# luicalrob/Triangulation-in-Deformable-Scenes

Measured on AMD Instinct MI355X. Metric: LM iterations/sec + ms/iter at 100k corr × 2 views; 1/2/4/8-GPU scaling, higher is better.
Workload: dtype f64

## Files before the change

### triangulation-in-deformable-scenes_amd/csrc/spcg.hip

```cpp
#include <hip/hip_runtime.h>

#include <algorithm>
#include <cstdio>
#include <type_traits>

#include "spcg.h"
#include "ticket.h"
#include "wave.h"

namespace deftri {
namespace sp {

using wv::wave_sum;
using wv::wave_max;

__device__ __forceinline__ double block_sum(double v, double *red4) {
    const int lane = threadIdx.x & 63, w = threadIdx.x >> 6;
    v = wave_sum(v);
    if (lane == 0) red4[w] = v;
    __syncthreads();
    const double s = (red4[0] + red4[1]) + (red4[2] + red4[3]);
    __syncthreads();
    return s;
}

__device__ __forceinline__ double pval(const double2 *__restrict__ zp, double beta, int64_t i) {
    const double2 v = zp[i];
    return __fma_rn(beta, v.y, v.x);
}

__device__ __forceinline__ int it_state(const SpDev &G, int it, double &beta) {
    beta = 0.0;
    if (G.rec[0] != 0.0) return (int)G.rec[0];
    const double *rk = G.red + (int64_t)kSpRed * it;
    if (rk[2] != 0.0) return (int)rk[2];
    if (rk[1] <= G.tol2 * G.red[1]) return kSpConverged;
    if (it >= G.max_it) return kSpBudget;
    if (it > 0) beta = rk[0] / G.red[(int64_t)kSpRed * (it - 1)];
    return 0;
}

__device__ __forceinline__ void record_stop(const SpDev &G, int it, int st) {
    if (G.rec[0] == 0.0) {
        G.rec[0] = st;
        G.rec[1] = it;
    }
}

__host__ __device__ __forceinline__ int row_grid(int nrb) { return 8 * ((max(nrb, 1) + 7) / 8); }
__device__ __forceinline__ int row_block(int b, int nrb) {
    const int seg = (max(nrb, 1) + 7) / 8;
    return (b & 7) * seg + (b >> 3);
}

__device__ __forceinline__ int heavy_dof(const SpDev &G, int h) { return h < G.Q ? 6 * h : 6 * G.Q + (h - G.Q); }

__device__ __forceinline__ bool gated_off(const int *g) { return g && !*g; }
__device__ __forceinline__ double lam_of(const SpDev &G, double lam) { return G.lam_dev ? *G.lam_dev : lam; }

__device__ __forceinline__ void publish(double *p, double v) { st_sc1(p, v); }
__device__ __forceinline__ double fetch(const double *p) {
    return ld_sc1(p);
}

__device__ __forceinline__ int tri3(int a, int b) { return a * (a + 1) / 2 + b; }
__device__ __forceinline__ int tri6(int a, int b) { return a * (a + 1) / 2 + b; }

template <class JT, int GU>
__global__ void __launch_bounds__(256) __attribute__((amdgpu_waves_per_eu(GU == 4 ? 5 : GU == 6 ? 4 : 1, GU == 4 ? 5 : GU == 6 ? 4 : 3)))
k_sp_glin_rows(const SpDev G, JT *__restrict__ pj) {
    __shared__ double red4[4];
    if (gated_off(G.lgate)) return;
    const int lb = row_block(blockIdx.x, G.nrb2);
    const int w = lb * 4 + (threadIdx.x >> 6), lane = threadIdx.x & 63;
    double mx = 0.0;
    if (w < G.nwaves) {
        const int l = G.rowmap[64 * w + lane];
        double D[6] = {0, 0, 0, 0, 0, 0}, bb[3] = {0, 0, 0};
        if (l >= 0) {
            for (int j = G.rep_off[l]; j < G.rep_off[l + 1]; j++) {
                const double *J = G.Jr + 6 * (int64_t)j;
                const double wt = G.Wr[j];
#pragma unroll
                for (int r = 0; r < 2; r++) {
                    const double er = G.Er[2 * (int64_t)j + r];
#pragma unroll
                    for (int a = 0; a < 3; a++) {
                        const double ja = J[3 * r + a] * wt;
#pragma unroll
                        for (int c = 0; c <= a; c++) D[tri3(a, c)] += ja * J[3 * r + c];
                        bb[a] -= J[3 * r + a] * (wt * er);
                    }
                }
            }
            const int d0 = G.dep_off[l], d1 = G.dep_off[l + 1];
            for (int jb = d0; jb < d1; jb += 4) {
                double Jb[4][4], wb[4], eb[4];
#pragma unroll
                for (int u = 0; u < 4; u++) {
                    const int64_t j = jb + u < d1 ? jb + u : jb;
#pragma unroll
                    for (int c = 0; c < 4; c++) Jb[u][c] = G.Jd[4 * j + c];
                    wb[u] = G.Wd[j];
                    eb[u] = G.Ed[j];
                }
#pragma unroll
                for (int u = 0; u < 4; u++) {
                    if (jb + u >= d1) break;
                    const int64_t j = jb + u;
                    const double *J = Jb[u];
                    const double wt = wb[u], er = eb[u];
#pragma unroll
                    for (int a = 0; a < 3; a++) {
                        const double ja = J[a] * wt;
#pragma unroll
                        for (int c = 0; c <= a; c++) D[tri3(a, c)] += ja * J[c];
                        bb[a] -= J[a] * (wt * er);
                        G.cdep[3 * j + a] = ja * J[3];
                    }
                    G.wss[j] = (J[3] * wt) * J[3];
                }
            }
        }
        double H[6];
#pragma unroll
        for (int k = 0; k < 6; k++) H[k] = D[k];
        const int64_t n = G.nslots * 64;
        struct Raw { double j0, j1, j2, w, x; };
        const double *__restrict__ Ja = G.Ja, *__restrict__ Wa = G.Wa, *__restrict__ Ea = G.Ea;
        const double *__restrict__ Jd = G.Jd, *__restrict__ Wd = G.Wd;
        const int64_t jld = G.jld;
        const bool w1 = G.Q == 1 && G.pinfo != nullptr;
        auto load = [&](int m) -> Raw {
            const bool dep = m <= -2;
            const int mm = max(m, 0), jj = max(-2 - m, 0);
            const double *pa = Ja + (int64_t)(3 * (mm & 3)) * jld + (mm >> 2);
            const double *pd = Jd + 4 * (int64_t)jj;
            const double *Jc = dep ? pd : pa;
            const int64_t st = dep ? 1 : jld;
            const double *W = dep ? Wd + jj : w1 ? G.pinfo : Wa + (mm >> 2);
            const double *X = dep ? pd + 3 : Ea + (mm >> 2);
            return Raw{Jc[0], Jc[st], Jc[2 * st], *W, *X};
        };
        auto value = [&](int m, const Raw &r, double *v, double &wt, double &er) {
            const bool arap = m >= 0, dep = m <= -2;
            v[0] = dep ? (r.j0 * r.w) * r.x : arap ? r.j0 : 0.0;
            v[1] = dep ? (r.j1 * r.w) * r.x : arap ? r.j1 : 0.0;
            v[2] = dep ? (r.j2 * r.w) * r.x : arap ? r.j2 : 0.0;
            wt = arap ? r.w : 0.0;
            er = arap ? r.x : 0.0;
        };
        auto add = [&](const double *v, double wt, double er) {
#pragma unroll
            for (int a = 0; a < 3; a++) {
                const double ja = v[a] * wt;
#pragma unroll
                for (int c = 0; c <= a; c++) H[tri3(a, c)] += ja * v[c];
                bb[a] -= v[a] * (wt * er);
            }
        };
        int64_t k = G.woff[w] * 64 + lane;
        const int64_t k1 = G.woff[w + 1] * 64 + lane;
        auto step = [&](auto U_, bool clamp) {
            constexpr int U = decltype(U_)::value;
            int m[U];
            int64_t kk[U];
            bool in[U];
            Raw r[U];
#pragma unroll
            for (int u = 0; u < U; u++) {
                in[u] = !clamp || k + 64 * u < k1;
                kk[u] = in[u] ? k + 64 * u : k1 - 64;
            }
#pragma unroll
            for (int u = 0; u < U; u++) m[u] = G.pmap[kk[u]];
#pragma unroll
            for (int u = 0; u < U; u++) r[u] = load(m[u]);
#pragma unroll
            for (int u = 0; u < U; u++) {
                double v[3], wt, er;
                value(m[u], r[u], v, wt, er);
                if (!in[u]) wt = er = 0.0;
                add(v, wt, er);
                if (pj)
#pragma unroll
                    for (int a = 0; a < 3; a++) pj[a * n + kk[u]] = (JT)v[a];
            }
            k += U * 64;
        };
        using I4 = std::integral_constant<int, 4>;
        if constexpr (GU == 4) {
            while (k + 3 * 64 < k1) step(I4{}, false);
        } else if constexpr (GU == 6) {
            while (k + 5 * 64 < k1) step(std::integral_constant<int, 6>{}, false);
            if (k + 4 * 64 < k1) step(std::integral_constant<int, 6>{}, true);
        } else {
            while (k + 7 * 64 < k1) step(std::integral_constant<int, 8>{}, false);
            if (k + 4 * 64 < k1) step(std::integral_constant<int, 8>{}, true);
        }
        if (k < k1) step(I4{}, true);
        if (G.wsplit[w]) {
#pragma unroll
            for (int k = 0; k < 6; k++) H[k] += __shfl_xor(H[k], 32);
#pragma unroll
            for (int a = 0; a < 3; a++) bb[a] += __shfl_xor(bb[a], 32);
        }
        if (l >= 0) {
#pragma unroll
            for (int k = 0; k < 6; k++) { G.Hv[6 * (int64_t)l + k] = H[k]; G.Dv[6 * (int64_t)l + k] = D[k]; }
            const int64_t o = G.hd + 3 * (int64_t)(G.row0 + l);
#pragma unroll
            for (int a = 0; a < 3; a++) G.b[o + a] = bb[a];
            mx = fmax(fabs(H[0]), fmax(fabs(H[2]), fabs(H[5])));
        }
    }
    mx = wave_max(mx);
    if ((threadIdx.x & 63) == 0) red4[threadIdx.x >> 6] = mx;
    __syncthreads();
    if (threadIdx.x == 0 && lb < max(G.nrb2, 1)) G.mpart[lb] = fmax(fmax(red4[0], red4[1]), fmax(red4[2], red4[3]));
}

__global__ void __launch_bounds__(256) k_sp_glin_blocks(const SpDev G) {
    __shared__ double red[kSpLin][4];
    if (gated_off(G.lgate)) return;
    const int2 gr = G.glb[blockIdx.x];
    const int4 d = G.blk[gr.x];
    const int kind = d.x & 0xff, owned = d.x >> 8;
    const int lane = threadIdx.x & 63, w = threadIdx.x >> 6;
    const int i = d.z + threadIdx.x;
    double *out = G.lpart + (int64_t)kSpLin * gr.x;
    if (kind == SP_ARAP) {
        if (!owned) return;
        double a[kSpLin];
#pragma unroll
        for (int k = 0; k < kSpLin; k++) a[k] = 0.0;
        const int iend = G.blk[gr.x + gr.y - 1].w;
        for (int ii = i; ii < iend; ii += 256) {
            double J[6];
#pragma unroll
            for (int r = 0; r < 6; r++) J[r] = G.Ja[(12 + r) * G.jld + ii];
            const double wv = G.Wa[ii], er = G.Ea[ii];
#pragma unroll
            for (int r = 0; r < 6; r++) {
                const double jr = J[r] * wv;
#pragma unroll
                for (int c = 0; c <= r; c++) a[tri6(r, c)] += jr * J[c];
                a[21 + r] -= J[r] * (wv * er);
            }
        }
        for (int k = threadIdx.x; k < kSpLin * (gr.y - 1); k += 256) out[kSpLin + k] = 0.0;
#pragma unroll
        for (int k = 0; k < kSpLin; k++) {
            const double v = wave_sum(a[k]);
            if (lane == 0) red[k][w] = v;
        }
        __syncthreads();
        if (threadIdx.x < kSpLin) {
            const int k = threadIdx.x;
            out[k] = (red[k][0] + red[k][1]) + (red[k][2] + red[k][3]);
        }
    } else {
        double h = 0.0, bs = 0.0;
        if (i < d.w) {
            const int le = G.dperm[i];
            const double js = G.Jd[4 * (int64_t)le + 3];
            h = G.wss[le];
            bs = -js * (G.Wd[le] * G.Ed[le]);
        }
        h = wave_sum(h);
        bs = wave_sum(bs);
        if (lane == 0) { red[0][w] = h; red[1][w] = bs; }
        __syncthreads();
        if (threadIdx.x < 2) {
            const int k = threadIdx.x;
            out[k] = (red[k][0] + red[k][1]) + (red[k][2] + red[k][3]);
        }
    }
}

__global__ void __launch_bounds__(256) k_sp_glin_heavy(const SpDev G) {
    __shared__ double lds[8][32];
    __shared__ int last;
    if (gated_off(G.lgate)) return;
    const int ch = blockIdx.x, h = G.ch_h[ch];
    const int dim = h < G.Q ? kSpLin : 2;
    const int c = threadIdx.x & 31, g = threadIdx.x >> 5;
    double acc = 0.0;
    if (c < dim) {
        int64_t k = G.ch_lo[ch] + g;
        const int64_t k1 = G.ch_lo[ch + 1];
        for (; k + 7 * 8 < k1; k += 64) {
            double v[8];
#pragma unroll
            for (int u = 0; u < 8; u++) v[u] = G.lpart[(int64_t)kSpLin * G.hv_blk[k + 8 * u] + c];
#pragma unroll
            for (int u = 0; u < 8; u++) acc += v[u];
        }
        for (; k < k1; k += 8) acc += G.lpart[(int64_t)kSpLin * G.hv_blk[k] + c];
    }
    lds[g][c] = acc;
    __syncthreads();
    if ((int)threadIdx.x < dim) {
        double t = 0.0;
#pragma unroll
        for (int gg = 0; gg < 8; gg++) t += lds[gg][threadIdx.x];
        publish(G.chpart + (int64_t)kSpLin * ch + threadIdx.x, t);
    }
    const int c0 = G.hch_off[h], c1 = G.hch_off[h + 1];
    if (threadIdx.x == 0) {
        __atomic_signal_fence(__ATOMIC_SEQ_CST);
        __builtin_amdgcn_s_waitcnt(0);
        __atomic_signal_fence(__ATOMIC_SEQ_CST);
        last = __hip_atomic_fetch_add(G.hcnt + h, 1, __ATOMIC_RELAXED, __HIP_MEMORY_SCOPE_AGENT) == c1 - c0 - 1;
    }
    __syncthreads();
    if (!last) return;
    acc = 0.0;
    if (c < dim)
        for (int j = c0 + g; j < c1; j += 8) acc += fetch(G.chpart + (int64_t)kSpLin * j + c);
    __syncthreads();
    lds[g][c] = acc;
    __syncthreads();
    if ((int)threadIdx.x < dim) {
        double t = 0.0;
#pragma unroll
        for (int gg = 0; gg < 8; gg++) t += lds[gg][threadIdx.x];
        const int q = threadIdx.x;
        if (h < G.Q) {
            if (q < 21) G.hl[21 * (int64_t)h + q] = t;
            else G.b[6 * (int64_t)h + q - 21] = t;
        } else {
            if (q == 0) G.hl[21 * (int64_t)G.Q + (h - G.Q)] = t;
            else G.b[6 * (int64_t)G.Q + (h - G.Q)] = t;
        }
    }
    if (threadIdx.x == 0) st_sc1(G.hcnt + h, 0);
}

__global__ void __launch_bounds__(256) k_sp_maxdiag(const SpDev G, double *out, int stage) {
    __shared__ double red4[4];
    if (gated_off(G.lgate)) return;
    double m = 0.0;
    if (stage == 0) {
        for (int i = threadIdx.x; i < G.nrb2; i += 256) m = fmax(m, G.mpart[i]);
    } else {
        for (int h = threadIdx.x; h < G.Q; h += 256)
#pragma unroll
            for (int a = 0; a < 6; a++) m = fmax(m, fabs(G.hl[21 * (int64_t)h + tri6(a, a)]));
        for (int s = threadIdx.x; s < G.S; s += 256) m = fmax(m, fabs(G.hl[21 * (int64_t)G.Q + s]));
    }
    m = wave_max(m);
    if ((threadIdx.x & 63) == 0) red4[threadIdx.x >> 6] = m;
    __syncthreads();
    if (threadIdx.x == 0) {
        const double v = fmax(fmax(red4[0], red4[1]), fmax(red4[2], red4[3]));
        out[0] = stage == 0 ? v : fmax(out[0], v);
    }
}

__global__ void k_sp_cvt_j(const double *__restrict__ J, float *__restrict__ J32, int64_t n, const int *gate) {
    if (gated_off(gate)) return;
    const int64_t i = (int64_t)blockIdx.x * 256 + threadIdx.x;
    if (i < n) J32[i] = (float)J[i];
}

__device__ __forceinline__ bool inv3(const double *A, double lam, double *M) {
    const double a00 = A[0] + lam, a10 = A[1], a11 = A[2] + lam, a20 = A[3], a21 = A[4], a22 = A[5] + lam;
    if (!(a00 > 0.0)) return false;
    const double l00 = sqrt(a00), l10 = a10 / l00, l20 = a20 / l00;
    const double d1 = a11 - l10 * l10;
    if (!(d1 > 0.0)) return false;
    const double l11 = sqrt(d1), l21 = (a21 - l20 * l10) / l11;
    const double d2 = a22 - l20 * l20 - l21 * l21;
    if (!(d2 > 0.0)) return false;
    const double l22 = sqrt(d2);
    const double i00 = 1.0 / l00, i11 = 1.0 / l11, i22 = 1.0 / l22;
    const double i10 = -l10 * i00 * i11;
    const double i21 = -l21 * i11 * i22;
    const double i20 = -(l20 * i00 + l21 * i10) * i22;
    M[0] = i00 * i00 + i10 * i10 + i20 * i20;
    M[1] = i11 * i10 + i21 * i20;
    M[2] = i11 * i11 + i21 * i21;
    M[3] = i22 * i20;
    M[4] = i22 * i21;
    M[5] = i22 * i22;
    return true;
}

__device__ __forceinline__ void mul3(const double *M, const double r[3], double z[3]) {
    z[0] = M[0] * r[0] + M[1] * r[1] + M[3] * r[2];
    z[1] = M[1] * r[0] + M[2] * r[1] + M[4] * r[2];
    z[2] = M[3] * r[0] + M[4] * r[1] + M[5] * r[2];
}

__device__ bool inv6(const double *Hl, double lam, double *Mo) {
    double L[36];
    for (int i = 0; i < 6; i++)
        for (int j = 0; j < 6; j++) L[i * 6 + j] = j <= i ? Hl[tri6(i, j)] + (i == j ? lam : 0.0) : 0.0;
    for (int j = 0; j < 6; j++) {
        double s = L[j * 6 + j];
        for (int k = 0; k < j; k++) s -= L[j * 6 + k] * L[j * 6 + k];
        if (!(s > 0.0)) return false;
        s = sqrt(s);
        L[j * 6 + j] = s;
        for (int i = j + 1; i < 6; i++) {
            double t = L[i * 6 + j];
            for (int k = 0; k < j; k++) t -= L[i * 6 + k] * L[j * 6 + k];
            L[i * 6 + j] = t / s;
        }
    }
    for (int c = 0; c < 6; c++) {
        double y[6];
        for (int i = 0; i < 6; i++) {
            double t = i == c ? 1.0 : 0.0;
            for (int k = 0; k < i; k++) t -= L[i * 6 + k] * y[k];
            y[i] = t / L[i * 6 + i];
        }
        for (int i = 5; i >= 0; i--) {
            double t = y[i];
            for (int k = i + 1; k < 6; k++) t -= L[k * 6 + i] * y[k];
// ... 845 lines not shown
                double z = 0.0;
                for (int c = 0; c < dim; c++) z += M[a * dim + c] * r[c];
                G.zp[o + a] = make_double2(z, p[a]);
                rz += r[a] * z;
                rr += r[a] * r[a];
            }
        }
        if (!G.include_heavy) rz = rr = 0.0;
    }
    rz = wave_sum(rz);
    rr = wave_sum(rr);
    if (lane == 0) { red[0][wv] = rz; red[1][wv] = rr; }
    __syncthreads();
    if (t == 0) {
        double s0 = 0.0, s1 = 0.0;
#pragma unroll
        for (int k = 0; k < nw; k++) { s0 += red[0][k]; s1 += red[1][k]; }
        double *out = G.upart + 2 * slot;
        if (G.fuse) {
            st_sc1(out, s0);
            st_sc1(out + 1, s1);
        } else {
            out[0] = s0;
            out[1] = s1;
        }
    }
    if (G.fuse && last_block(G, G.cnt + 16)) {
        __syncthreads();
        if (t < 256) dots_block(G, it + 1, dred);
    }
}

__global__ void __launch_bounds__(3 * kSpUpdRows) k_sp_update_sd(int it, const SpDev G, double lam, int tail) {
    __shared__ double sM[6 * kSpUpdRows], sR[3 * kSpUpdRows];
    __shared__ double red[2][3 * kSpUpdRows / 64];
    if (gated_off(G.gate) || G.rec[0] != 0.0) return;
    lam = lam_of(G, lam);
    const double gamma = G.xb[0], rr = G.xb[1], delta = G.xb[2];
    const double rr0 = it == 0 ? rr : G.red[1];
    double beta = 0.0, alpha = 0.0;
    int st = 0;
    if (rr <= G.tol2 * rr0) st = kSpConverged;
    else if (it >= G.max_it) st = kSpBudget;
    else {
        double den = delta;
        if (it > 0) {
            beta = gamma / G.red[(int64_t)kSpRed * (it - 1)];
            den = delta - beta * gamma / G.red[(int64_t)kSpRed * (it - 1) + 3];
        }
        alpha = gamma / den;
        if (!(den > 0.0) || !isfinite(alpha) || !isfinite(beta)) st = kSpBreakdown;
    }
    const int t = threadIdx.x, lane = t & 63, wv = t >> 6;
    if (blockIdx.x == 0 && t == 0) {
        double *rk = G.red + (int64_t)kSpRed * it;
        rk[0] = gamma; rk[1] = rr; rk[3] = alpha; rk[4] = delta;
        if (st) record_stop(G, it, st);
    }
    if (st || tail) return;
    constexpr int nw = 3 * kSpUpdRows / 64;
    double rz = 0.0, rr1 = 0.0;
    const int rb = (int)blockIdx.x - 1, slot = rb < 0 ? G.nrb : rb;
    if (rb >= 0) {
        const int l0 = rb * kSpUpdRows;
        const int nrow = min(kSpUpdRows, G.nown - l0);
        const int64_t o0 = G.hd + 3 * (int64_t)(G.row0 + l0);
        const bool on = t < 3 * nrow;
        double z = 0.0, pp = 0.0, w = 0.0, sp = 0.0, x = 0.0, r = 0.0;
        if (on) {
            const double2 v = G.zp[o0 + t];
            z = v.x; pp = v.y;
            w = G.q[o0 + t];
            if (G.tile) {
                const int l = l0 + t / 3, a = t - 3 * (t / 3);
                for (int k = G.txoff[l]; k < G.txoff[l + 1]; k++) w += G.xc[3 * (int64_t)k + a];
            }
            sp = G.sv[o0 + t];
            x = G.x[o0 + t];
            r = G.r[o0 + t];
        }
        const double *Mg = G.Mv + 6 * (int64_t)l0;
        if (t < 6 * nrow) sM[t] = Mg[t];
        if (t + 3 * kSpUpdRows < 6 * nrow) sM[t + 3 * kSpUpdRows] = Mg[t + 3 * kSpUpdRows];
        const double p = it > 0 ? z + beta * pp : z;
        const double s_ = it > 0 ? w + beta * sp : w;
        x += alpha * p;
        r -= alpha * s_;
        sR[t] = r;
        __syncthreads();
        if (on) {
            const int row = t / 3, a = t - 3 * row;
            const double *M = sM + 6 * row, *rv = sR + 3 * row;
            const int i0 = a == 0 ? 0 : a == 1 ? 1 : 3, i1 = a == 0 ? 1 : a == 1 ? 2 : 4, i2 = a == 0 ? 3 : a == 1 ? 4 : 5;
            const double zn = M[i0] * rv[0] + M[i1] * rv[1] + M[i2] * rv[2];
            G.x[o0 + t] = x;
            G.r[o0 + t] = r;
            G.sv[o0 + t] = s_;
            G.zp[o0 + t] = make_double2(zn, p);
            sd_send(G, l0 + row, a, zn, p);
            rz = r * zn;
            rr1 = r * r;
        }
    } else if (t < 256) {
        for (int h = t; h < G.Q + G.S; h += 256) {
            const int o = heavy_dof(G, h);
            const int dim = h < G.Q ? 6 : 1;
            double r[6], p[6];
            for (int a = 0; a < dim; a++) {
                const double2 v = G.zp[o + a];
                const double w = G.xb[3 + o + a] + lam * v.x;
                p[a] = it > 0 ? v.x + beta * v.y : v.x;
                const double s_ = it > 0 ? w + beta * G.sv[o + a] : w;
                G.sv[o + a] = s_;
                G.x[o + a] += alpha * p[a];
                r[a] = G.r[o + a] - alpha * s_;
                G.r[o + a] = r[a];
            }
            const double *M = h < G.Q ? G.Mh + 36 * (int64_t)h : G.Mh + 36 * (int64_t)G.Q + (h - G.Q);
            for (int a = 0; a < dim; a++) {
                double z = 0.0;
                for (int c = 0; c < dim; c++) z += M[a * dim + c] * r[c];
                G.zp[o + a] = make_double2(z, p[a]);
                rz += r[a] * z;
                rr1 += r[a] * r[a];
            }
        }
        if (!G.include_heavy) rz = rr1 = 0.0;
    }
    rz = wave_sum(rz);
    rr1 = wave_sum(rr1);
    if (lane == 0) { red[0][wv] = rz; red[1][wv] = rr1; }
    __syncthreads();
    if (t == 0) {
        double s0 = 0.0, s1 = 0.0;
#pragma unroll
        for (int k = 0; k < nw; k++) { s0 += red[0][k]; s1 += red[1][k]; }
        G.upart[2 * slot] = s0;
        G.upart[2 * slot + 1] = s1;
    }
}

__device__ __forceinline__ double shfl_up_d(double v, int d) {
    int2 p = __builtin_bit_cast(int2, v);
    p.x = __shfl_up(p.x, (unsigned)d, 64);
    p.y = __shfl_up(p.y, (unsigned)d, 64);
    return __builtin_bit_cast(double, p);
}

__device__ __forceinline__ int tile_state(const SpDev &G, int it, double &beta, double (*red)[4]) {
    beta = 0.0;
    __shared__ double s_r0;
    const double *rk = G.red + (int64_t)kSpRed * it;
    const double sw = rk[2], rr0 = G.red[1], gprev = it > 0 ? G.red[(int64_t)kSpRed * (it - 1)] : 1.0;
    if (threadIdx.x == 0) s_r0 = G.rec[0];
    __syncthreads();
    const double r0 = s_r0;
    if (r0 != 0.0) return (int)r0;
    const int n2 = it == 0 ? G.nrb + 1 : G.m_nh + row_grid(G.nrb);
    const double2 *parts = reinterpret_cast<const double2 *>(it == 0 ? G.upart : G.m2part);
    double a0 = 0.0, a1 = 0.0;
    int j = (int)threadIdx.x;
    for (; j + 3 * 256 < n2; j += 4 * 256) {
        double2 v[4];
#pragma unroll
        for (int u = 0; u < 4; u++) v[u] = parts[j + 256 * u];
#pragma unroll
        for (int u = 0; u < 4; u++) { a0 += v[u].x; a1 += v[u].y; }
    }
    for (; j < n2; j += 256) {
        const double2 v = parts[j];
        a0 += v.x;
        a1 += v.y;
    }
    const int lane = threadIdx.x & 63, w = threadIdx.x >> 6;
    a0 = wave_sum(a0);
    a1 = wave_sum(a1);
    if (lane == 0) { red[0][w] = a0; red[1][w] = a1; }
    __syncthreads();
    const double s0 = (red[0][0] + red[0][1]) + (red[0][2] + red[0][3]);
    const double s1 = (red[1][0] + red[1][1]) + (red[1][2] + red[1][3]);
    __syncthreads();
    int st = 0;
    if (sw != 0.0) st = (int)sw;
    else if (s1 <= G.tol2 * (it == 0 ? s1 : rr0)) st = kSpConverged;
    else if (it >= G.max_it) st = kSpBudget;
    if (blockIdx.x == 0 && threadIdx.x == 0) {
        G.red[(int64_t)kSpRed * it] = s0;
        G.red[(int64_t)kSpRed * it + 1] = s1;
        if (st) record_stop(G, it, st);
    }
    if (!st && it > 0) beta = s0 / gprev;
    return st;
}

__device__ __forceinline__ double tile_heavy_sum(const SpDev &G, int h, double *lds, bool coherent = false) {
    const int nb = G.t_grid - 1;
    const int dim = h < G.Q ? 6 : 1;
    const int c = threadIdx.x & 7, g = threadIdx.x >> 3;
    double acc = 0.0;
    if (G.tmulti) {
        const int q = h < G.Q ? h : (h - G.Q) >> 1, off = h < G.Q ? 0 : 6 + ((h - G.Q) & 1);
        const int seg = (G.ntile + 7) / 8, t1 = G.tpoff[q + 1];
        if (c < dim)
            for (int t = G.tpoff[q] + g; t < t1; t += 32) {
                const double *p = G.part + (int64_t)kSpPart * (8 * (t % seg) + t / seg) + off + c;
                acc += coherent ? fetch(p) : *p;
            }
    } else if (c < dim) {
        const int off = h < G.Q ? 0 : 6 + (h - G.Q);
        int k = g;
        for (; k + 7 * 32 < nb; k += 8 * 32) {
            double v[8];
#pragma unroll
            for (int u = 0; u < 8; u++) {
                const double *q = G.part + (int64_t)kSpPart * (k + 32 * u) + off + c;
                v[u] = coherent ? fetch(q) : *q;
            }
#pragma unroll
            for (int u = 0; u < 8; u++) acc += v[u];
        }
        for (; k < nb; k += 32) {
            const double *q = G.part + (int64_t)kSpPart * k + off + c;
            acc += coherent ? fetch(q) : *q;
        }
    }
    lds[threadIdx.x] = acc;
    __syncthreads();
    double t = 0.0;
    if ((int)threadIdx.x < dim)
        for (int gg = 0; gg < 32; gg++) t += lds[8 * gg + threadIdx.x];
    return t;
}

template <class JT, int SD = 0>
__global__ void __launch_bounds__(256) k_sp_tile(int it, const SpDev G, const JT *__restrict__ Jarap, double lam) {
    extern __shared__ double lds[];
    __shared__ double red[9][4];
    if (gated_off(G.gate)) return;
    lam = lam_of(G, lam);
    const int b = G.p1list ? G.p1list[blockIdx.x] : (int)blockIdx.x, tid = (int)threadIdx.x, lane = tid & 63, wv = tid >> 6;
    const bool heavy_wg = b == G.t_grid - 1;
    const int seg = (G.ntile + 7) / 8;
    const int t = heavy_wg ? G.ntile : (b & 7) * seg + (b >> 3);
    int r0 = 0, nr = 0, nh = 0, e0 = 0, ne = 0, h0 = 0, ns = 0, tq = 0;
    auto own_row = [&](int i) { return G.tmulti ? (G.trow[r0 + i] & 0x7fffffff) : G.row0 + r0 + i; };
    double2 zpre[3] = {make_double2(0.0, 0.0), make_double2(0.0, 0.0), make_double2(0.0, 0.0)};
    double2 zpre2[3] = {make_double2(0.0, 0.0), make_double2(0.0, 0.0), make_double2(0.0, 0.0)};
    double2 hz = make_double2(0.0, 0.0);
    uint2 mA = make_uint2(0u, 0u), mB = mA;
    int2 cA = make_int2(0, 0), cB = cA;
    int rsi = 0, dj0 = 0, dj1 = 0;
    int dsc0 = -1;
    double cd0[3] = {0.0, 0.0, 0.0}, ws0 = 0.0, Dp[6] = {0, 0, 0, 0, 0, 0};
    if (t < G.ntile) {
        const int32_t *T = G.ttab + 8 * (int64_t)t;
        r0 = T[0]; nr = T[1]; nh = T[2]; e0 = T[3]; ne = T[4]; h0 = T[5]; ns = T[6]; tq = T[7];
        if (tid < nr + nh) {
            const int row = tid < nr ? own_row(tid) : G.thalo[h0 + tid - nr];
            const int64_t o = G.hd + 3 * (int64_t)row;
#pragma unroll
            for (int c = 0; c < 3; c++) zpre[c] = G.zp[o + c];
        }
        if (tid + 256 < nr + nh) {
            const int i = tid + 256;
            const int row = i < nr ? own_row(i) : G.thalo[h0 + i - nr];
            const int64_t o = G.hd + 3 * (int64_t)row;
#pragma unroll
            for (int c = 0; c < 3; c++) zpre2[c] = G.zp[o + c];
        }
        const int hdof = tid < 6 ? 6 * tq + tid : 6 * G.Q + 2 * tq + tid - 6;
        if (tid < 8 && hdof < G.hd) hz = G.zp[hdof];
        const int64_t k0 = (int64_t)e0 + tid;
        if (tid < ne) { mA = G.tmeta[k0]; cA = G.tchunk[k0 >> 6]; }
        if (tid + 256 < ne) { mB = G.tmeta[k0 + 256]; cB = G.tchunk[(k0 + 256) >> 6]; }
        if (tid < nr) {
            const int l = G.tmulti ? own_row(tid) : r0 + tid;
            rsi = G.trs[r0 + tid];
            if (G.tmulti) {
                const int tdv = G.tdep[r0 + tid];
                if (tdv >= 0) {
                    const int jd = tdv >> 1;
                    dsc0 = tdv & 1;
#pragma unroll
                    for (int c = 0; c < 3; c++) cd0[c] = G.cdep[3 * (int64_t)jd + c];
                    ws0 = G.wss[jd];
                }
                if (G.trow[r0 + tid] < 0)
#pragma unroll
                    for (int kk = 0; kk < 6; kk++) Dp[kk] = G.Dv[6 * (int64_t)l + kk];
            } else {
                dj0 = G.dep_off[l];
                dj1 = G.dep_off[l + 1];
            }
        }
    }
    double beta;
    if (G.sd) {
        beta = 0.0;
        if (G.rec[0] != 0.0) return;
    } else if (G.tparts) {
        if (tile_state(G, it, beta, reinterpret_cast<double(*)[4]>(&red[0][0]))) return;
    } else if (it_state(G, it, beta)) {
        return;
    }
    double pap = 0.0, jts[6] = {0, 0, 0, 0, 0, 0}, sacc[2] = {0, 0};
    if (heavy_wg) {
        for (int64_t dd = tid; dd < G.hd; dd += 256) {
            const double p = pval(G.zp, beta, dd);
            G.ph[dd] = p;
            pap += lam * (p * p);
        }
        if (!G.include_heavy) pap = 0.0;
        pap = block_sum(pap, red[0]);
        if (tid == 0) G.m1part[b] = pap;
        return;
    }
    if (t < G.ntile) {
        double *pL = lds, *up = pL + 3 * (nr + nh), *rs = up + 3 * nr, *hp = rs + 3 * ns;
        const int64_t jld = G.jld;
        const uint64_t lt = (1ull << lane) - 1;
        if (tid < nr + nh)
#pragma unroll
            for (int c = 0; c < 3; c++) pL[3 * tid + c] = __fma_rn(beta, zpre[c].y, zpre[c].x);
        if (tid + 256 < nr + nh)
#pragma unroll
// ... 215 lines not shown
                    for (int u = 0; u < 4; u++)
                        if (j0 + u < ns)
#pragma unroll
                            for (int c = 0; c < 3; c++) q[c] += v[u][c];
                }
            }
            {
                const int k0 = G.txoff[l], k1 = G.txoff[l + 1];
                for (int kb = k0; kb < k1; kb += 4) {
                    double v[4][3];
#pragma unroll
                    for (int u = 0; u < 4; u++) {
                        const int64_t k = kb + u < k1 ? kb + u : kb;
#pragma unroll
                        for (int c = 0; c < 3; c++) v[u][c] = G.xc[3 * k + c];
                    }
#pragma unroll
                    for (int u = 0; u < 4; u++)
                        if (kb + u < k1)
#pragma unroll
                            for (int c = 0; c < 3; c++) q[c] += v[u][c];
                }
            }
            if (FIN) {
#pragma unroll
                for (int c = 0; c < 3; c++) G.q[o + c] = q[c];
            } else {
#pragma unroll
                for (int c = 0; c < 3; c++) {
                    const double2 v = G.zp[o + c];
                    pr[c] = __fma_rn(beta, v.y, v.x);
                    xo[c] = G.x[o + c];
                    ro[c] = G.r[o + c];
                }
#pragma unroll
                for (int k = 0; k < 6; k++) M[k] = G.Mv[6 * (int64_t)l + k];
            }
        }
        if (!FIN && !own_alpha && !G.alpha_kernel) alpha = m2_alpha_wait(G, it);
        if (!FIN && on && !isnan(alpha)) {
            double r[3], z[3];
#pragma unroll
            for (int c = 0; c < 3; c++) {
                G.x[o + c] = xo[c] + alpha * pr[c];
                r[c] = ro[c] - alpha * q[c];
            }
            z[0] = M[0] * r[0] + M[1] * r[1] + M[3] * r[2];
            z[1] = M[1] * r[0] + M[2] * r[1] + M[4] * r[2];
            z[2] = M[3] * r[0] + M[4] * r[1] + M[5] * r[2];
#pragma unroll
            for (int c = 0; c < 3; c++) {
                G.r[o + c] = r[c];
                G.zp[o + c] = make_double2(z[c], pr[c]);
                pq += r[c] * z[c];
                rr2 += r[c] * r[c];
            }
        }
    }
    if (FIN) return;
    __shared__ double red[2][4];
    if (G.tparts && !last) {
        pair_tree(pq, rr2, red, G.m2part + 2 * blockIdx.x, 0);
        return;
    }
    pair_tree(pq, rr2, red, G.m2part + 2 * blockIdx.x, 1);
    m2_dots(G, it, red);
}

__global__ void __launch_bounds__(256) k_sp_txb(int it, const SpDev G) {
    __shared__ double red4[4];
    __shared__ double lds[256];
    (void)it;
    if (gated_off(G.gate) || G.rec[0] != 0.0) return;
    const int nh = G.Q + G.S, h = (int)blockIdx.x;
    if (h < nh) {
        const double t = tile_heavy_sum(G, h, lds);
        if ((int)threadIdx.x < (h < G.Q ? 6 : 1)) G.xb[3 + heavy_dof(G, h) + threadIdx.x] = t;
    } else if (h == nh) {
        double a = 0.0;
        for (int j = threadIdx.x; j < G.t_grid; j += 256) a += G.m1part[j];
        a = block_sum(a, red4);
        if (threadIdx.x == 0) G.xb[2] = a;
    } else {
        double a0 = 0.0, a1 = 0.0;
        for (int j = threadIdx.x; j <= G.nrb; j += 256) { a0 += G.upart[2 * j]; a1 += G.upart[2 * j + 1]; }
        a0 = block_sum(a0, red4);
        a1 = block_sum(a1, red4);
        if (threadIdx.x == 0) { G.xb[0] = a0; G.xb[1] = a1; }
    }
}


__global__ void k_sp_pack(int n, const int32_t *__restrict__ rows, int width, int64_t base, const double *__restrict__ src,
                          double *__restrict__ buf) {
    const int64_t t = (int64_t)blockIdx.x * 256 + threadIdx.x;
    if (t >= (int64_t)n * width) return;
    const int64_t i = t / width, c = t % width;
    buf[t] = src[base + (int64_t)width * rows[i] + c];
}

__global__ void k_sp_unpack(int n, const int32_t *__restrict__ rows, int width, int64_t base, const double *__restrict__ buf,
                            double *__restrict__ dst) {
    const int64_t t = (int64_t)blockIdx.x * 256 + threadIdx.x;
    if (t >= (int64_t)n * width) return;
    const int64_t i = t / width, c = t % width;
    dst[base + (int64_t)width * rows[i] + c] = buf[t];
}

__global__ void k_sp_load_p(int64_t n, const double *__restrict__ v, double2 *__restrict__ zp) {
    const int64_t t = (int64_t)blockIdx.x * 256 + threadIdx.x;
    if (t < n) zp[t] = make_double2(v[t], 0.0);
}

__global__ void k_sp_permute(int32_t P, int64_t hd, const int32_t *__restrict__ row_of_point, const double *__restrict__ src,
                             double *__restrict__ dst, int to_plan) {
    const int64_t t = (int64_t)blockIdx.x * 256 + threadIdx.x;
    if (t < hd) { dst[t] = src[t]; return; }
    const int64_t u = t - hd;
    if (u >= 3 * (int64_t)P) return;
    const int64_t pt = u / 3, c = u % 3;
    const int64_t row = row_of_point[pt];
    if (to_plan) dst[hd + 3 * row + c] = src[hd + 3 * pt + c];
    else dst[hd + 3 * pt + c] = src[hd + 3 * row + c];
}

}

static inline unsigned nblk(int64_t n, int bs) { return (unsigned)std::max<int64_t>((n + bs - 1) / bs, 1); }

#define SPL(NAME, KER, GRID, ...)                                          \
    do {                                                                   \
        if ((GRID) <= 0) break;                               \
        hipEvent_t e0_ = prof_begin(st);                                   \
        hipLaunchKernelGGL(KER, dim3(GRID), dim3(256), 0, st, __VA_ARGS__); \
        prof_end(NAME, e0_, (unsigned)(GRID), 0.0, st);                    \
    } while (0)

#define SPLS(NAME, KER, GRID, LDS, ...)                                              \
    do {                                                                             \
        if ((GRID) <= 0) break;                                                      \
        hipEvent_t e0_ = prof_begin(st);                                             \
        hipLaunchKernelGGL(KER, dim3(GRID), dim3(256), (size_t)(LDS), st, __VA_ARGS__); \
        prof_end(NAME, e0_, (unsigned)(GRID), 0.0, st);                              \
    } while (0)

template <class JT, int MG>
static void launch_phase2(const SpDev &G, int grid, int it, double lambda, const JT *pj, hipStream_t st) {
    if (G.p2u == 4) SPL("sp_phase2", (sp::k_sp_phase2<JT, MG, 4>), grid, it, G, lambda, pj);
    else if (G.p2u == 6) SPL("sp_phase2", (sp::k_sp_phase2<JT, MG, 6>), grid, it, G, lambda, pj);
    else SPL("sp_phase2", (sp::k_sp_phase2<JT, MG, 8>), grid, it, G, lambda, pj);
}

void sp_launch_glin(const SpDev &G, bool fp32, hipStream_t st) {
    if (G.glu == 4) {
        if (fp32) SPL("sp_glin_rows", (sp::k_sp_glin_rows<float, 4>), sp::row_grid(G.nrb2), G, G.pj32);
        else SPL("sp_glin_rows", (sp::k_sp_glin_rows<double, 4>), sp::row_grid(G.nrb2), G, G.pj);
    } else if (G.glu == 6) {
        if (fp32) SPL("sp_glin_rows", (sp::k_sp_glin_rows<float, 6>), sp::row_grid(G.nrb2), G, G.pj32);
        else SPL("sp_glin_rows", (sp::k_sp_glin_rows<double, 6>), sp::row_grid(G.nrb2), G, G.pj);
    } else {
        if (fp32) SPL("sp_glin_rows", (sp::k_sp_glin_rows<float, 8>), sp::row_grid(G.nrb2), G, G.pj32);
        else SPL("sp_glin_rows", (sp::k_sp_glin_rows<double, 8>), sp::row_grid(G.nrb2), G, G.pj);
    }
    if (G.nblk > 0) SPL("sp_glin_blocks", sp::k_sp_glin_blocks, G.nglb, G);
    if (G.nch > 0) SPL("sp_glin_heavy", sp::k_sp_glin_heavy, G.nch, G);
}

void sp_launch_maxdiag(const SpDev &G, double *out, hipStream_t st) {
    SPL("sp_maxdiag", sp::k_sp_maxdiag, 1, G, out, 0);
}

void sp_launch_maxdiag_heavy(const SpDev &G, double *out, hipStream_t st) {
    SPL("sp_maxdiag", sp::k_sp_maxdiag, 1, G, out, 1);
}

void sp_launch_cvt_j(const double *J, float *J32, int64_t n, hipStream_t st, const int *gate) {
    if (n > 0) SPL("sp_cvt_j", sp::k_sp_cvt_j, nblk(n, 256), J, J32, n, gate);
}

void sp_launch_setup(const SpDev &G, const double *rhs, double lambda, hipStream_t st) {
    const int grid = (G.nown + kSpUpdRows - 1) / kSpUpdRows + 1;
    hipEvent_t e0_ = prof_begin(st);
    hipLaunchKernelGGL(sp::k_sp_setup, dim3(grid), dim3(3 * kSpUpdRows), 0, st, G, rhs, lambda);
    prof_end("sp_setup", e0_, (unsigned)grid, 0.0, st);
}

void sp_launch_dots(const SpDev &G, int it, hipStream_t st) {
    SPL("sp_dots", sp::k_sp_dots, 1, it, G);
}

void sp_launch_product(const SpDev &G, int it, double lambda, bool fp32, hipStream_t st, bool last) {
    if (G.sd) {
        sp_launch_sd_phase1(G, it, lambda, fp32, st, nullptr, sp_merged_grid1(G));
        sp_launch_sd_phase2(G, it, lambda, fp32, st);
        return;
    }
    if (G.tile) {
        hipEvent_t e0_ = prof_begin(st);
        if (fp32) hipLaunchKernelGGL((sp::k_sp_tile<float>), dim3(G.t_grid), dim3(256), (size_t)G.tile_lds, st, it, G, G.Ja32, lambda);
        else hipLaunchKernelGGL((sp::k_sp_tile<double>), dim3(G.t_grid), dim3(256), (size_t)G.tile_lds, st, it, G, G.Ja, lambda);
        prof_end("sp_tile", e0_, (unsigned)G.t_grid, 0.0, st);
        if (G.alpha_kernel) SPL("sp_alpha", sp::k_sp_alpha, 1, it, G);
        SPL("sp_tupd", (sp::k_sp_tupd<0>), G.m_nh + sp::row_grid(G.nrb), it, G, lambda, last ? 1 : 0);
        return;
    }
    if (G.merged) {
        const int g1 = sp_merged_grid1(G), g2 = sp_merged_grid2(G);
        if (fp32) SPL("sp_phase1", (sp::k_sp_phase1<float, 1>), g1, it, G, G.Ja32, lambda);
        else SPL("sp_phase1", (sp::k_sp_phase1<double, 1>), g1, it, G, G.Ja, lambda);
        if (G.alpha_kernel) SPL("sp_alpha", sp::k_sp_alpha, 1, it, G);
        if (fp32) launch_phase2<float, 1>(G, g2, it, lambda, G.pj32, st);
        else launch_phase2<double, 1>(G, g2, it, lambda, G.pj, st);
        return;
    }
    if (G.nblk > 0) {
        if (fp32) SPL("sp_phase1", (sp::k_sp_phase1<float, 0>), G.nblk, it, G, G.Ja32, lambda);
        else SPL("sp_phase1", (sp::k_sp_phase1<double, 0>), G.nblk, it, G, G.Ja, lambda);
    }
    const int grid = sp::row_grid(G.nrb2) + (G.fuse_heavy ? G.Q + G.S : 0);
    if (fp32) launch_phase2<float, 0>(G, grid, it, lambda, G.pj32, st);
    else launch_phase2<double, 0>(G, grid, it, lambda, G.pj, st);
}

void sp_launch_tile_sd(const SpDev &G, int it, double lambda, bool fp32, hipStream_t st, const int32_t *list, int n,
                       bool txb) {
    if (n > 0) {
        SpDev g = G;
        g.p1list = list;
        hipEvent_t e0_ = prof_begin(st);
        if (fp32) hipLaunchKernelGGL((sp::k_sp_tile<float, 1>), dim3(n), dim3(256), (size_t)G.tile_lds, st, it, g, G.Ja32, lambda);
        else hipLaunchKernelGGL((sp::k_sp_tile<double, 1>), dim3(n), dim3(256), (size_t)G.tile_lds, st, it, g, G.Ja, lambda);
        prof_end("sp_tile", e0_, (unsigned)n, 0.0, st);
    }
    if (txb) SPL("sp_txb", sp::k_sp_txb, G.Q + G.S + 2, it, G);
}

void sp_launch_tile_product(const SpDev &G, double lambda, bool fp32, hipStream_t st) {
    hipEvent_t e0_ = prof_begin(st);
    if (fp32) hipLaunchKernelGGL((sp::k_sp_tile<float>), dim3(G.t_grid), dim3(256), (size_t)G.tile_lds, st, 0, G, G.Ja32, lambda);
    else hipLaunchKernelGGL((sp::k_sp_tile<double>), dim3(G.t_grid), dim3(256), (size_t)G.tile_lds, st, 0, G, G.Ja, lambda);
    prof_end("sp_tile", e0_, (unsigned)G.t_grid, 0.0, st);
    SPL("sp_tupd", (sp::k_sp_tupd<1>), G.m_nh + sp::row_grid(G.nrb), 0, G, lambda, 1);
}

int sp_merged_grid1(const SpDev &G) { return 8 * ((G.nrb + 1 + 7) / 8) + G.nblk; }

void sp_launch_sd_phase1(const SpDev &G, int it, double lambda, bool fp32, hipStream_t st, const int32_t *list, int n) {
    SpDev g = G;
    g.p1list = list;
    if (fp32) SPL("sp_phase1", (sp::k_sp_phase1<float, 2>), n, it, g, G.Ja32, lambda);
    else SPL("sp_phase1", (sp::k_sp_phase1<double, 2>), n, it, g, G.Ja, lambda);
}

void sp_launch_sd_phase2(const SpDev &G, int it, double lambda, bool fp32, hipStream_t st) {
    const int g2 = G.m_nh + sp::row_grid(G.nrb2);
    if (fp32) launch_phase2<float, 2>(G, g2, it, lambda, G.pj32, st);
    else launch_phase2<double, 2>(G, g2, it, lambda, G.pj, st);
}
int sp_merged_grid2(const SpDev &G) { return 8 * ((G.Q + G.S + 7) / 8) + sp::row_grid(G.nrb2); }

void sp_launch_heavy(const SpDev &G, int it, double lambda, int stage, hipStream_t st) {
    const int grid = (stage == 1 && G.heavy_split) ? G.Q + G.S + 1 : 1;
    SPL("sp_heavy", sp::k_sp_heavy, grid, it, G, lambda, stage);
}

void sp_launch_update_sd(const SpDev &G, int it, double lambda, int tail, hipStream_t st) {
    const int grid = (G.nown + kSpUpdRows - 1) / kSpUpdRows + 1;
    hipEvent_t e0_ = prof_begin(st);
    hipLaunchKernelGGL(sp::k_sp_update_sd, dim3(grid), dim3(3 * kSpUpdRows), 0, st, it, G, lambda, tail);
    prof_end("sp_update", e0_, (unsigned)grid, 0.0, st);
}

void sp_launch_update(const SpDev &G, int it, hipStream_t st) {
    const int grid = (G.nown + kSpUpdRows - 1) / kSpUpdRows + 1;
    hipEvent_t e0_ = prof_begin(st);
    hipLaunchKernelGGL(sp::k_sp_update, dim3(grid), dim3(3 * kSpUpdRows), 0, st, it, G);
    prof_end("sp_update", e0_, (unsigned)grid, 0.0, st);
}

void sp_launch_halo_pack(int n, const int32_t *rows, int width, int64_t base, const double *src, double *buf,
                         hipStream_t st) {
    if (n > 0) SPL("sp_halo_pack", sp::k_sp_pack, nblk((int64_t)n * width, 256), n, rows, width, base, src, buf);
}

void sp_launch_halo_unpack(int n, const int32_t *rows, int width, int64_t base, const double *buf, double *dst,
                           hipStream_t st) {
    if (n > 0) SPL("sp_halo_unpack", sp::k_sp_unpack, nblk((int64_t)n * width, 256), n, rows, width, base, buf, dst);
}

void sp_launch_load_p(int64_t n, const double *v, double2 *zp, hipStream_t st) {
    SPL("sp_load_p", sp::k_sp_load_p, nblk(n, 256), n, v, zp);
}

void sp_launch_permute_in(int32_t P, int64_t hd, const int32_t *row_of_point, const double *src, double *dst,
                          hipStream_t st) {
    SPL("sp_permute", sp::k_sp_permute, nblk(hd + 3 * (int64_t)P, 256), P, hd, row_of_point, src, dst, 1);
}

void sp_launch_permute_out(int32_t P, int64_t hd, const int32_t *row_of_point, const double *src, double *dst,
                           hipStream_t st) {
    SPL("sp_permute", sp::k_sp_permute, nblk(hd + 3 * (int64_t)P, 256), P, hd, row_of_point, src, dst, 0);
}

}
```

Baseline: 1762.

## Fuse glin block kernel into rows kernel and prefetch CG partials before sync

The separate sp_glin_blocks launch is folded into k_sp_glin_rows as a leading range of blocks, with the block count padded to a multiple of 8 so the row_block interleaving stays aligned. This removes one kernel launch per linearization. The diagonal-block Hessian term is now recomputed from Jd and Wd instead of read from the precomputed wss array. In tile_state, the first partial-sum loads are issued before the rec[0] barrier so their latency overlaps the sync. The fused kernel carries the extra shared array and branch, which may affect register and occupancy tuning of the rows kernel.

```diff
diff --git a/triangulation-in-deformable-scenes_amd/csrc/spcg.hip b/triangulation-in-deformable-scenes_amd/csrc/spcg.hip
--- a/triangulation-in-deformable-scenes_amd/csrc/spcg.hip
+++ b/triangulation-in-deformable-scenes_amd/csrc/spcg.hip
@@ -66,12 +66,17 @@
 __device__ __forceinline__ int tri3(int a, int b) { return a * (a + 1) / 2 + b; }
 __device__ __forceinline__ int tri6(int a, int b) { return a * (a + 1) / 2 + b; }
 
+__device__ __forceinline__ void glin_blocks(const SpDev &G, int bid);
 template <class JT, int GU>
 __global__ void __launch_bounds__(256) __attribute__((amdgpu_waves_per_eu(GU == 4 ? 5 : GU == 6 ? 4 : 1, GU == 4 ? 5 : GU == 6 ? 4 : 3)))
-k_sp_glin_rows(const SpDev G, JT *__restrict__ pj) {
+k_sp_glin_rows(const SpDev G, JT *__restrict__ pj, int nbw) {
     __shared__ double red4[4];
     if (gated_off(G.lgate)) return;
-    const int lb = row_block(blockIdx.x, G.nrb2);
+    if ((int)blockIdx.x < nbw) {
+        glin_blocks(G, (int)blockIdx.x);
+        return;
+    }
+    const int lb = row_block((int)blockIdx.x - nbw, G.nrb2);
     const int w = lb * 4 + (threadIdx.x >> 6), lane = threadIdx.x & 63;
     double mx = 0.0;
     if (w < G.nwaves) {
@@ -220,10 +225,10 @@
     if (threadIdx.x == 0 && lb < max(G.nrb2, 1)) G.mpart[lb] = fmax(fmax(red4[0], red4[1]), fmax(red4[2], red4[3]));
 }
 
-__global__ void __launch_bounds__(256) k_sp_glin_blocks(const SpDev G) {
+__device__ __forceinline__ void glin_blocks(const SpDev &G, int bid) {
     __shared__ double red[kSpLin][4];
-    if (gated_off(G.lgate)) return;
-    const int2 gr = G.glb[blockIdx.x];
+    if (bid >= G.nglb) return;
+    const int2 gr = G.glb[bid];
     const int4 d = G.blk[gr.x];
     const int kind = d.x & 0xff, owned = d.x >> 8;
     const int lane = threadIdx.x & 63, w = threadIdx.x >> 6;
@@ -264,8 +269,9 @@
         if (i < d.w) {
             const int le = G.dperm[i];
             const double js = G.Jd[4 * (int64_t)le + 3];
-            h = G.wss[le];
-            bs = -js * (G.Wd[le] * G.Ed[le]);
+            const double wt = G.Wd[le];
+            h = (js * wt) * js;
+            bs = -js * (wt * G.Ed[le]);
         }
         h = wave_sum(h);
         bs = wave_sum(bs);
@@ -1417,25 +1423,25 @@
     __shared__ double s_r0;
     const double *rk = G.red + (int64_t)kSpRed * it;
     const double sw = rk[2], rr0 = G.red[1], gprev = it > 0 ? G.red[(int64_t)kSpRed * (it - 1)] : 1.0;
-    if (threadIdx.x == 0) s_r0 = G.rec[0];
-    __syncthreads();
-    const double r0 = s_r0;
-    if (r0 != 0.0) return (int)r0;
     const int n2 = it == 0 ? G.nrb + 1 : G.m_nh + row_grid(G.nrb);
     const double2 *parts = reinterpret_cast<const double2 *>(it == 0 ? G.upart : G.m2part);
     double a0 = 0.0, a1 = 0.0;
     int j = (int)threadIdx.x;
-    for (; j + 3 * 256 < n2; j += 4 * 256) {
-        double2 v[4];
-#pragma unroll
-        for (int u = 0; u < 4; u++) v[u] = parts[j + 256 * u];
-#pragma unroll
-        for (int u = 0; u < 4; u++) { a0 += v[u].x; a1 += v[u].y; }
-    }
-    for (; j < n2; j += 256) {
-        const double2 v = parts[j];
-        a0 += v.x;
-        a1 += v.y;
+    double2 v[4];
+#pragma unroll
+    for (int u = 0; u < 4; u++) v[u] = j + 256 * u < n2 ? parts[j + 256 * u] : make_double2(0.0, 0.0);
+    if (threadIdx.x == 0) s_r0 = G.rec[0];
+    __syncthreads();
+    const double r0 = s_r0;
+    if (r0 != 0.0) return (int)r0;
+    for (;;) {
+#pragma unroll
+        for (int u = 0; u < 4; u++)
+            if (j + 256 * u < n2) { a0 += v[u].x; a1 += v[u].y; }
+        j += 4 * 256;
+        if (j >= n2) break;
+#pragma unroll
+        for (int u = 0; u < 4; u++) v[u] = j + 256 * u < n2 ? parts[j + 256 * u] : make_double2(0.0, 0.0);
     }
     const int lane = threadIdx.x & 63, w = threadIdx.x >> 6;
     a0 = wave_sum(a0);
@@ -1957,17 +1963,17 @@
 }
 
 void sp_launch_glin(const SpDev &G, bool fp32, hipStream_t st) {
+    const int nbw = G.nblk > 0 ? 8 * ((G.nglb + 7) / 8) : 0, grid = nbw + sp::row_grid(G.nrb2);
     if (G.glu == 4) {
-        if (fp32) SPL("sp_glin_rows", (sp::k_sp_glin_rows<float, 4>), sp::row_grid(G.nrb2), G, G.pj32);
-        else SPL("sp_glin_rows", (sp::k_sp_glin_rows<double, 4>), sp::row_grid(G.nrb2), G, G.pj);
+        if (fp32) SPL("sp_glin_rows", (sp::k_sp_glin_rows<float, 4>), grid, G, G.pj32, nbw);
+        else SPL("sp_glin_rows", (sp::k_sp_glin_rows<double, 4>), grid, G, G.pj, nbw);
     } else if (G.glu == 6) {
-        if (fp32) SPL("sp_glin_rows", (sp::k_sp_glin_rows<float, 6>), sp::row_grid(G.nrb2), G, G.pj32);
-        else SPL("sp_glin_rows", (sp::k_sp_glin_rows<double, 6>), sp::row_grid(G.nrb2), G, G.pj);
+        if (fp32) SPL("sp_glin_rows", (sp::k_sp_glin_rows<float, 6>), grid, G, G.pj32, nbw);
+        else SPL("sp_glin_rows", (sp::k_sp_glin_rows<double, 6>), grid, G, G.pj, nbw);
     } else {
-        if (fp32) SPL("sp_glin_rows", (sp::k_sp_glin_rows<float, 8>), sp::row_grid(G.nrb2), G, G.pj32);
-        else SPL("sp_glin_rows", (sp::k_sp_glin_rows<double, 8>), sp::row_grid(G.nrb2), G, G.pj);
-    }
-    if (G.nblk > 0) SPL("sp_glin_blocks", sp::k_sp_glin_blocks, G.nglb, G);
+        if (fp32) SPL("sp_glin_rows", (sp::k_sp_glin_rows<float, 8>), grid, G, G.pj32, nbw);
+        else SPL("sp_glin_rows", (sp::k_sp_glin_rows<double, 8>), grid, G, G.pj, nbw);
+    }
     if (G.nch > 0) SPL("sp_glin_heavy", sp::k_sp_glin_heavy, G.nch, G);
 }
 
```

After: 1782 (median of 4 runs). No clear change (+1.2%).
